# tiberiu44/TTS-Cube

Hardware: AMD Instinct MI355X
Metric: audio samples/sec (HiFi-GAN vocoder inference) (higher is better)
Workload: dtype f32 (split fp16 hi/lo x3 MFMA, fp32 accumulate)

## Files before the change

include/ttscube_hip.h:

```cpp
#ifndef TTSCUBE_HIP_H
#define TTSCUBE_HIP_H

#include <stddef.h>
#include <stdint.h>

#ifdef __cplusplus
extern "C" {
#endif

#define TTSC_OK 0
#define TTSC_EINVAL (-1)
#define TTSC_EHIP (-2)
#define TTSC_ESTATE (-3)
#define TTSC_ENOMEM (-4)
#define TTSC_ERANGE (-5)

const char* ttsc_version(void);
const char* ttsc_last_error(void);
int ttsc_device_count(void);

typedef struct ttsc_conv1d ttsc_conv1d;

typedef struct {
    int32_t in_channels;
// ... 18 lines not shown
    const float* gate_dev;
    float gate_slope;
} ttsc_conv1d_epilogue;

int ttsc_conv1d_create(const ttsc_conv1d_cfg* cfg, ttsc_conv1d** out);
int ttsc_conv1d_set_weight(ttsc_conv1d* c, const float* weight_host, const float* bias_host);
int ttsc_conv1d_set_weight_device(ttsc_conv1d* c, const float* weight_dev, const float* bias_dev, void* stream);
int ttsc_conv1d_set_weight_device_dgrad(ttsc_conv1d* c, const float* fwd_weight_dev, void* stream);
int ttsc_conv1d_set_precision(ttsc_conv1d* c, int32_t precision);
int64_t ttsc_conv1d_out_len(const ttsc_conv1d* c, int64_t Lin);
int32_t ttsc_conv1d_in_channels(const ttsc_conv1d* c);
int ttsc_conv1d_set_activation_scale(ttsc_conv1d* c, float scale);
float ttsc_conv1d_get_activation_scale(const ttsc_conv1d* c);
int ttsc_conv1d_set_nonfinite_flag(ttsc_conv1d* c, uint32_t* flag_dev);
int ttsc_absmax(const float* x_dev, int64_t n, float* out_dev, void* stream);
int ttsc_conv1d_forward(const ttsc_conv1d* c, const float* x_dev, int32_t B, int64_t Lin, float* y_dev,
                        const float* resid_dev, const ttsc_conv1d_epilogue* ep, void* stream);
int ttsc_conv1d_forward_ragged(const ttsc_conv1d* c, const float* x_dev, int32_t B, int64_t Lin, float* y_dev,
                               const float* resid_dev, const ttsc_conv1d_epilogue* ep, const int32_t* in_len_dev,
                               const int32_t* out_len_dev, void* stream);
int ttsc_conv1d_forward_pitched(const ttsc_conv1d* c, const float* x_dev, int32_t B, int64_t Lin, float* y_dev,
                                const float* resid_dev, const ttsc_conv1d_epilogue* ep, const int32_t* in_len_dev,
                                const int32_t* out_len_dev, int64_t Lout_pitch, void* stream);
int ttsc_respair_supported(const ttsc_conv1d* conv1, const ttsc_conv1d* conv2);
int ttsc_respair_forward(const ttsc_conv1d* conv1, const ttsc_conv1d* conv2, const float* x_dev, int32_t B, int64_t L,
                         float* y_dev, int32_t accumulate, const int32_t* len_dev, void* stream);
int ttsc_rbchain_supported(const ttsc_conv1d* const* convs1, const ttsc_conv1d* const* convs2, int32_t npairs);
int ttsc_rbchain_forward(const ttsc_conv1d* const* convs1, const ttsc_conv1d* const* convs2, int32_t npairs, const float* x_dev,
                         int32_t B, int64_t L, float* y_dev, int32_t accumulate, const int32_t* len_dev, int32_t tile_shape,
                         void* stream);
int ttsc_rbchain_post_supported(const ttsc_conv1d* const* convs1, const ttsc_conv1d* const* convs2, int32_t npairs, const ttsc_conv1d* post);
int ttsc_rbchain_post_forward(const ttsc_conv1d* const* convs1, const ttsc_conv1d* const* convs2, int32_t npairs, const float* x_dev, int32_t B,
                              int64_t L, const float* ysum_dev, const ttsc_conv1d* post, const ttsc_conv1d_epilogue* post_ep, float* wav_dev,
                              const int32_t* len_dev, void* stream);
void ttsc_conv1d_destroy(ttsc_conv1d* c);

int ttsc_weight_norm_forward(const float* v_dev, const float* g_dev, float* w_dev, float* norm_dev, int32_t rows, int64_t cols, void* stream);
int ttsc_weight_norm_backward(const float* dw_dev, const float* v_dev, const float* g_dev, const float* norm_dev, float* dv_dev,
                              float* dg_dev, int32_t rows, int64_t cols, void* stream);
size_t ttsc_matvec_workspace_bytes(int32_t rows, int64_t cols);
int ttsc_matvec(const float* w_dev, int32_t rows, int64_t cols, const float* x_dev, int32_t transpose, float* out_dev, void* ws_dev, size_t ws_bytes,
                void* stream);
int ttsc_l2_normalize(const float* x_dev, int32_t n, float eps, float* out_dev, float* norm_dev, void* stream);
size_t ttsc_dot_workspace_bytes(int64_t n);
int ttsc_dot(const float* a_dev, const float* b_dev, int64_t n, float* out_dev, void* ws_dev, size_t ws_bytes, void* stream);
int ttsc_div_scalar(const float* w_dev, const float* sigma_dev, float* out_dev, int64_t n, void* stream);
// ... 334 lines not shown
```

ttscube_amd/_lib.py:

```python
import ctypes as C
import os

_HERE = os.path.dirname(os.path.abspath(__file__))
LIB_PATH = os.path.join(_HERE, 'csrc', 'libttscube_hip.so')


class TTSCError(RuntimeError):
    pass


class Conv1dCfg(C.Structure):
    _fields_ = [('in_channels', C.c_int32), ('out_channels', C.c_int32), ('kernel_size', C.c_int32),
                ('stride', C.c_int32), ('padding', C.c_int32), ('dilation', C.c_int32), ('transposed', C.c_int32), ('groups', C.c_int32)]


class Conv1dEpilogue(C.Structure):
    _fields_ = [('in_scale', C.c_float), ('in_slope', C.c_float), ('out_scale', C.c_float),
                ('out_act', C.c_int32), ('accumulate', C.c_int32), ('gate_dev', C.c_void_p), ('gate_slope', C.c_float)]


MAX_UPS, MAX_RB, MAX_DIL = 8, 8, 8


class WBankEntry(C.Structure):
# ... 44 lines not shown
    'ttsc_device_count': (C.c_int, []),
    'ttsc_conv1d_create': (C.c_int, [C.POINTER(Conv1dCfg), C.POINTER(C.c_void_p)]),
    'ttsc_conv1d_set_weight': (C.c_int, [C.c_void_p, C.c_void_p, C.c_void_p]),
    'ttsc_conv1d_set_precision': (C.c_int, [C.c_void_p, C.c_int32]),
    'ttsc_conv1d_out_len': (C.c_int64, [C.c_void_p, C.c_int64]),
    'ttsc_conv1d_set_activation_scale': (C.c_int, [C.c_void_p, C.c_float]),
    'ttsc_conv1d_get_activation_scale': (C.c_float, [C.c_void_p]),
    'ttsc_absmax': (C.c_int, [C.c_void_p, C.c_int64, C.c_void_p, C.c_void_p]),
    'ttsc_hifigan_calibrate': (C.c_int, [C.c_void_p, C.c_void_p, C.c_int32, C.c_int64, C.c_void_p, C.c_void_p, C.c_size_t, C.c_void_p]),
    'ttsc_hifigan_get_activation_scale': (C.c_int, [C.c_void_p, C.c_char_p, C.POINTER(C.c_float)]),
    'ttsc_hifigan_set_activation_scales': (C.c_int, [C.c_void_p, C.POINTER(C.c_char_p), C.POINTER(C.c_float), C.c_int32]),
    'ttsc_hifigan_recalibrations': (C.c_int32, [C.c_void_p]),
    'ttsc_hifigan_set_branch_streams': (C.c_int, [C.c_void_p, C.c_void_p, C.c_void_p]),
    'ttsc_hifigan_set_range_check': (C.c_int, [C.c_void_p, C.c_int32]),
    'ttsc_hifigan_range_status': (C.c_int32, [C.c_void_p, C.c_void_p]),
    'ttsc_conv1d_set_nonfinite_flag': (C.c_int, [C.c_void_p, C.c_void_p]),
    'ttsc_conv1d_in_channels': (C.c_int32, [C.c_void_p]),
    'ttsc_conv1d_forward': (C.c_int, [C.c_void_p, C.c_void_p, C.c_int32, C.c_int64, C.c_void_p, C.c_void_p,
                                      C.POINTER(Conv1dEpilogue), C.c_void_p]),
    'ttsc_conv1d_forward_ragged': (C.c_int, [C.c_void_p, C.c_void_p, C.c_int32, C.c_int64, C.c_void_p, C.c_void_p,
                                             C.POINTER(Conv1dEpilogue), C.c_void_p, C.c_void_p, C.c_void_p]),
    'ttsc_conv1d_forward_pitched': (C.c_int, [C.c_void_p, C.c_void_p, C.c_int32, C.c_int64, C.c_void_p, C.c_void_p,
                                              C.POINTER(Conv1dEpilogue), C.c_void_p, C.c_void_p, C.c_int64, C.c_void_p]),
    'ttsc_rbchain_supported': (C.c_int, [C.POINTER(C.c_void_p), C.POINTER(C.c_void_p), C.c_int32]),
    'ttsc_rbchain_forward': (C.c_int, [C.POINTER(C.c_void_p), C.POINTER(C.c_void_p), C.c_int32, C.c_void_p, C.c_int32, C.c_int64,
                                       C.c_void_p, C.c_int32, C.c_void_p, C.c_int32, C.c_void_p]),
    'ttsc_rbchain_post_supported': (C.c_int, [C.POINTER(C.c_void_p), C.POINTER(C.c_void_p), C.c_int32, C.c_void_p]),
    'ttsc_rbchain_post_forward': (C.c_int, [C.POINTER(C.c_void_p), C.POINTER(C.c_void_p), C.c_int32, C.c_void_p, C.c_int32, C.c_int64, C.c_void_p,
                                            C.c_void_p, C.POINTER(Conv1dEpilogue), C.c_void_p, C.c_void_p, C.c_void_p]),
    'ttsc_respair_supported': (C.c_int, [C.c_void_p, C.c_void_p]),
    'ttsc_respair_forward': (C.c_int, [C.c_void_p, C.c_void_p, C.c_void_p, C.c_int32, C.c_int64, C.c_void_p, C.c_int32,
                                       C.c_void_p, C.c_void_p]),
    'ttsc_conv1d_destroy': (None, [C.c_void_p]),
    'ttsc_conv1d_set_weight_device': (C.c_int, [C.c_void_p, C.c_void_p, C.c_void_p, C.c_void_p]),
    'ttsc_conv_wgrad_grouped': (C.c_int, [C.c_void_p, C.c_void_p, C.c_void_p, C.c_int32, C.c_int32, C.c_int32, C.c_int32, C.c_int64, C.c_int64,
                                          C.c_int32, C.c_int32, C.c_int32, C.c_float, C.c_float, C.c_void_p, C.c_size_t, C.c_void_p]),
    'ttsc_conv_wgrad': (C.c_int, [C.c_void_p, C.c_void_p, C.c_void_p, C.c_int32, C.c_int32, C.c_int32, C.c_int64, C.c_int64,
                                  C.c_int32, C.c_int32, C.c_int32, C.c_float, C.c_float, C.c_void_p, C.c_size_t, C.c_void_p]),
    'ttsc_conv1d_set_weight_device_dgrad': (C.c_int, [C.c_void_p, C.c_void_p, C.c_void_p]),
    'ttsc_weight_norm_forward': (C.c_int, [C.c_void_p, C.c_void_p, C.c_void_p, C.c_void_p, C.c_int32, C.c_int64, C.c_void_p]),
    'ttsc_weight_norm_backward': (C.c_int, [C.c_void_p, C.c_void_p, C.c_void_p, C.c_void_p, C.c_void_p, C.c_void_p, C.c_int32,
                                            C.c_int64, C.c_void_p]),
    'ttsc_matvec_workspace_bytes': (C.c_size_t, [C.c_int32, C.c_int64]),
    'ttsc_matvec': (C.c_int, [C.c_void_p, C.c_int32, C.c_int64, C.c_void_p, C.c_int32, C.c_void_p, C.c_void_p, C.c_size_t, C.c_void_p]),
    'ttsc_rows_segment_sum': (C.c_int, [C.c_void_p, C.c_void_p, C.c_void_p, C.c_int64, C.c_int32, C.c_int32, C.c_void_p]),
    'ttsc_l2_normalize': (C.c_int, [C.c_void_p, C.c_int32, C.c_float, C.c_void_p, C.c_void_p, C.c_void_p]),
# ... 356 lines not shown
```

ttscube_amd/csrc/conv1d.hip:

```cpp
#include <climits>
#include <cmath>
#include <cstdlib>
#include <type_traits>

#include "common.hpp"
#include "conv_kernels.hpp"

namespace ttsc {

static constexpr unsigned LEAN_OOB = 0x80000000u;
__device__ __forceinline__ float lean_load(__amdgpu_buffer_rsrc_t rs, unsigned voff, int soff) {
    return __uint_as_float(__builtin_amdgcn_raw_buffer_load_b32(rs, (int)voff, soff, 0));
}

template <int C, int K, int D, bool LEAN>
__global__ __launch_bounds__(256, 2) void conv_f16x3_wide_kernel(ConvArgs a) {
    extern __shared__ __attribute__((aligned(16))) char smem_raw[];
    constexpr int WM = 2, WN = 2;
    constexpr int MI = 2, NJ = 4, NT = WN * NJ * 32;
    constexpr int SPAN = NT + (K - 1) * D;
    constexpr int SPANP = (SPAN + 63) & ~63;
    constexpr int BUFSZ = 4 * SPAN + 2;
    constexpr int NCHUNK = C / 16, COTN = C / 32;
    constexpr int AITEMS = WM * MI * 2 * 64;
    half8* Xp = reinterpret_cast<half8*>(smem_raw);
    half8* Aw = Xp + 2 * BUFSZ;
    const int tid = threadIdx.x, lane = tid & 63, wave = tid >> 6;
    const int wm = wave / WN, wn = wave % WN;
    const int half = lane >> 5, l31 = lane & 31;
    const int b = blockIdx.z;
    const int q0 = blockIdx.x * NT;
    const int lin = a.in_len ? a.in_len[b] : a.Lin;
    if (a.out_len && q0 >= a.out_len[b]) return;
    const int cotg = blockIdx.y * (WM * MI);
#ifdef TTSC_ABLATE
    const unsigned wg_lin = blockIdx.x + gridDim.x * (blockIdx.y + gridDim.y * blockIdx.z);
#endif
    TTSC_STAMP(a, wg_lin, 0);
    TTSC_STAMP_HWID(a, wg_lin, 15);

    f32x16 acc[MI][NJ];
    const float* ai_first = a.acc_init ? (a.resid ? a.resid : (a.accumulate ? a.y : nullptr)) : nullptr;
    const float* ai_second = (a.acc_init && a.resid && a.accumulate) ? a.y : nullptr;
    const unsigned ai_L = (unsigned)a.Lout;
    const unsigned ai_row0 = ((unsigned)b * a.Cout + (cotg + wm * MI) * 32 + 4 * half) * ai_L;
// ... 41 lines not shown
#pragma unroll
                        for (int r = 0; r < 16; ++r) acc[i][n0 + n][r] += t[n][r];
                }
        }
        if (a.bias) {
#pragma unroll
            for (int i = 0; i < MI; ++i) {
                float bv[16];
#pragma unroll
                for (int r = 0; r < 16; ++r) bv[r] = a.bias[(cotg + wm * MI + i) * 32 + (r & 3) + 8 * (r >> 2) + 4 * half];
#pragma unroll
                for (int n = 0; n < NJ; ++n)
#pragma unroll
                    for (int r = 0; r < 16; ++r) acc[i][n][r] += bv[r];
            }
        }
#pragma unroll
        for (int i = 0; i < MI; ++i)
#pragma unroll
            for (int n = 0; n < NJ; ++n)
#pragma unroll
                for (int r = 0; r < 16; ++r) acc[i][n][r] *= inv;
    };
    if (a.acc_init) {
    } else if (a.epi_prefetch && a.bias && (a.resid || a.accumulate)) {
        const float inv = 1.f / a.w_unscale;
#pragma unroll
        for (int i = 0; i < MI; ++i)
#pragma unroll
            for (int r = 0; r < 16; ++r) {
                const float bv = a.bias[(cotg + wm * MI + i) * 32 + (r & 3) + 8 * (r >> 2) + 4 * half] * inv;
#pragma unroll
                for (int j = 0; j < NJ; ++j) acc[i][j][r] = bv;
            }
    } else {
#pragma unroll
        for (int i = 0; i < MI; ++i)
#pragma unroll
            for (int j = 0; j < NJ; ++j)
#pragma unroll
                for (int r = 0; r < 16; ++r) acc[i][j][r] = 0.f;
    }

    const float* xb = a.x + (size_t)b * C * a.Lin;
    const int lo = q0 - D * ((K - 1) / 2);
    const half8* wsrc = reinterpret_cast<const half8*>(a.wph) + (size_t)cotg * 128 + lane;
    if (a.skew) {
// ... 9 lines not shown
        for (int i = 0; i < AITEMS / 64 / 4; ++i) {
            const int blk = wave + i * 4;
            __builtin_amdgcn_global_load_lds((const __attribute__((address_space(1))) void*)(wj + blk * 64),
                                             (__attribute__((address_space(3))) void*)(Aw + slot * AITEMS + blk * 64), 16, 0, 0);
        }
    };

    constexpr int XIT = (2 * SPANP + 255) / 256;
    static_assert(XIT <= K, "one staging item per tap");
    float xr[XIT][8];
    unsigned xoff[XIT];
    int xslot[XIT];
    bool xok[XIT];
#pragma unroll
    for (int e = 0; e < XIT; ++e) {
        const int i = tid + e * 256;
        const int h = i >= SPANP ? 1 : 0;
        const int p = i - h * SPANP;
        const int pos = lo + p;
        xok[e] = pos >= 0 && pos < lin;
        int pc = pos > lin - 1 ? lin - 1 : pos;
        pc = pc < 0 ? 0 : pc;
        xoff[e] = (unsigned)(h * 8 * a.Lin + pc);
        xslot[e] = (p < SPAN && i < 2 * SPANP) ? (h * 2) * SPAN + p : 4 * SPAN;
        if (LEAN) xoff[e] = (xok[e] && xslot[e] < 4 * SPAN) ? xoff[e] * 4u : LEAN_OOB;
    }
    const __amdgpu_buffer_rsrc_t xrs = __builtin_amdgcn_make_buffer_rsrc(const_cast<float*>(xb), 0, LEAN ? C * a.Lin * 4 : 0, 0x00020000);
    const int xrow = a.Lin * 4;
    auto x_issue_item = [&](int e, int c) __attribute__((always_inline)) {
        if constexpr (LEAN) {
            const int s0 = c * 16 * xrow;
#pragma unroll
            for (int ch = 0; ch < 8; ++ch) xr[e][ch] = lean_load(xrs, xoff[e], s0 + ch * xrow);
        } else {
            const float* rc = xb + (size_t)(c * 16) * a.Lin;
#pragma unroll
            for (int ch = 0; ch < 8; ++ch) xr[e][ch] = rc[(size_t)ch * a.Lin + xoff[e]];
        }
    };
    auto x_commit_item = [&](int e, half8* buf) __attribute__((always_inline)) {
        typedef unsigned u32x4 __attribute__((ext_vector_type(4)));
        u32x4 uh, ul;
#pragma unroll
        for (int ch = 0; ch < 8; ch += 2) {
            float v0 = (LEAN || xok[e]) ? xr[e][ch] * a.in_scale : 0.f, v1 = (LEAN || xok[e]) ? xr[e][ch + 1] * a.in_scale : 0.f;
            v0 = fmaxf(v0, v0 * a.in_slope);
            v1 = fmaxf(v1, v1 * a.in_slope);
            unsigned h, l;
            split2_f16(v0, v1, h, l);
            uh[ch >> 1] = h;
            ul[ch >> 1] = l;
        }
        const half8 vh = __builtin_bit_cast(half8, uh), vl = __builtin_bit_cast(half8, ul);
        buf[xslot[e]] = vh;
        buf[xslot[e] + (xslot[e] < 4 * SPAN ? SPAN : 1)] = vl;
    };

    const half8* xbase = Xp + (unsigned)((half * 2) * SPAN + wn * (NJ * 32) + l31);
    const half8* abase = Aw + (unsigned)(wm * (MI * 128) + lane);
    auto chunk = [&](int c, auto buf_tag, auto par_tag) __attribute__((always_inline)) {
        constexpr int BUF = decltype(buf_tag)::value;
        constexpr int PAR = decltype(par_tag)::value;
        half8* nxt = Xp + (1 - BUF) * BUFSZ;
#pragma unroll
        for (int j = 0; j < K; ++j) {
            const int slot = (PAR + j) & 1;
            if (j + 1 < K)
                stage_A(c, j + 1, slot ^ 1);
            else
                stage_A(c + 1 < NCHUNK ? c + 1 : c, 0, slot ^ 1);
            __builtin_amdgcn_sched_barrier(0);
            half8 ah[MI], al[MI], bh[NJ], bl[NJ];
#pragma unroll
            for (int i = 0; i < MI; ++i) {
                ah[i] = abase[slot * AITEMS + i * 128];
                al[i] = abase[slot * AITEMS + i * 128 + 64];
            }
#pragma unroll
            for (int n = 0; n < NJ; ++n) {
                bh[n] = xbase[BUF * BUFSZ + j * D + n * 32];
                bl[n] = xbase[BUF * BUFSZ + SPAN + j * D + n * 32];
            }
            const int e = K - 1 - j;
            if (e < XIT && !TTSC_DBG(a, 1)) {
                x_commit_item(e, nxt);
                x_issue_item(e, c + 2 < NCHUNK ? c + 2 : NCHUNK - 1);
            }
#pragma unroll
            for (int i = 0; i < MI; ++i)
#pragma unroll
                for (int n = 0; n < NJ; ++n) acc[i][n] = __builtin_amdgcn_mfma_f32_32x32x16_f16(al[i], bh[n], acc[i][n], 0, 0, 0);
#pragma unroll
            for (int i = 0; i < MI; ++i)
#pragma unroll
                for (int n = 0; n < NJ; ++n) acc[i][n] = __builtin_amdgcn_mfma_f32_32x32x16_f16(ah[i], bl[n], acc[i][n], 0, 0, 0);
#pragma unroll
            for (int i = 0; i < MI; ++i)
#pragma unroll
                for (int n = 0; n < NJ; ++n) acc[i][n] = __builtin_amdgcn_mfma_f32_32x32x16_f16(ah[i], bh[n], acc[i][n], 0, 0, 0);
            __builtin_amdgcn_sched_barrier(0);
            if (!TTSC_DBG(a, 2)) __syncthreads();
        }
    };

    stage_A(0, 0, 0);
#pragma unroll
    for (int e = 0; e < XIT; ++e) x_issue_item(e, 0);
    if (a.acc_init) {
        __builtin_amdgcn_sched_barrier(0);
        acc_load_first(0);
        __builtin_amdgcn_sched_barrier(0);
    }
#pragma unroll
    for (int e = 0; e < XIT; ++e) x_commit_item(e, Xp);
#pragma unroll
    for (int e = 0; e < XIT; ++e) x_issue_item(e, 1);
    if (a.acc_init) {
        __builtin_amdgcn_sched_barrier(0);
#pragma unroll
        for (int i = 1; i < MI; ++i) acc_load_first(i);
        acc_init_finish();
    }
    __syncthreads();
    TTSC_STAMP(a, wg_lin, 1);
    for (int c = 0; c < NCHUNK; c += 2) {
        chunk(c, std::integral_constant<int, 0>(), std::integral_constant<int, 0>());
        chunk(c + 1, std::integral_constant<int, 1>(), std::integral_constant<int, (K & 1)>());
    }
    TTSC_STAMP(a, wg_lin, 2);

    if (TTSC_DBG(a, 4)) {
        float t = 0.f;
#pragma unroll
        for (int i = 0; i < MI; ++i)
#pragma unroll
            for (int n = 0; n < NJ; ++n) t += acc[i][n][0] + acc[i][n][7];
        if (t == 12345.678f) a.y[0] = 1.f;
        return;
    }
    if (a.acc_init) {
#pragma unroll
        for (int i = 0; i < MI; ++i)
#pragma unroll
            for (int n = 0; n < NJ; ++n) {
                const int q = q0 + wn * (NJ * 32) + n * 32 + l31;
                if (q < a.Lout) {
                    float* yp = a.y + ((size_t)b * a.Cout + (cotg + wm * MI + i) * 32 + 4 * half) * a.Lout + q;
#pragma unroll
                    for (int r = 0; r < 16; ++r) yp[(size_t)((r & 3) + 8 * (r >> 2)) * a.Lout] = acc[i][n][r] * a.w_unscale;
                }
            }
    } else if (a.epi_prefetch && (a.resid || a.accumulate)) {
        const float* rsrc = a.resid;
        const float* ysrc = a.accumulate ? a.y : nullptr;
        constexpr int NTILE = MI * NJ;
        const unsigned L1 = (unsigned)a.Lout;
        const unsigned row0 = ((unsigned)b * a.Cout + (cotg + wm * MI) * 32 + 4 * half) * L1;
        const int qw = q0 + wn * (NJ * 32) + l31;
        auto tile_off = [&](int t) __attribute__((always_inline)) -> unsigned {
            const int i = t / NJ, n = t % NJ;
            const int q = qw + n * 32;
            return row0 + (unsigned)(i * 32) * L1 + (unsigned)(q < a.Lout ? q : 0);
        };
// ... 333 lines not shown
    } else {
#pragma unroll
        for (int e = 0; e < 4; ++e)
            if (q + e < a.Lout) yb[q + e] = res[e];
    }
}

template <int MI, int NJ, int TMAX>
static int launch_f16_t(const ConvArgs& a, int B, hipStream_t s) {
    constexpr int NT = 4 * NJ * 32;
    constexpr int MT = MI * 32;
    dim3 grid((unsigned)ceil_div(a.q_cnt, NT), (unsigned)(a.CoutP / MT), (unsigned)B);
    const size_t lds = (size_t)a.span_pad * 4 * 16 + (size_t)a.ntaps * MI * 2 * 64 * 16;
    if (int rc = ensure_full_lds((const void*)conv_f16x3_kernel<MI, NJ, TMAX>)) return rc;
    hipLaunchKernelGGL((conv_f16x3_kernel<MI, NJ, TMAX>), grid, dim3(256), lds, s, a);
    hipError_t e = hipGetLastError();
    if (e != hipSuccess) {
        set_error("conv_f16x3_kernel launch failed: %s", hipGetErrorString(e));
        return TTSC_EHIP;
    }
    return TTSC_OK;
}

template <int C, int K, int D, bool LEAN>
static int launch_f16_wide_l(const ConvArgs& a0, int B, hipStream_t s) {
    constexpr int NT = 256;
    constexpr int SPAN = NT + (K - 1) * D;
    dim3 grid((unsigned)ceil_div(a0.Lout, NT), (unsigned)(C / 128), (unsigned)B);
    ConvArgs a = a0;
    static const int skew_env = getenv("TTSC_CONV_SKEW") ? atoi(getenv("TTSC_CONV_SKEW")) : 0;
    a.skew = ((size_t)grid.x * grid.y * grid.z >= 1024) ? skew_env : 0;
    static const int epi_env = getenv("TTSC_CONV_EPI_PREFETCH") ? atoi(getenv("TTSC_CONV_EPI_PREFETCH")) : 1;
    a.epi_prefetch = (epi_env && !a.gate && a.out_act == TTSC_ACT_NONE && a.Cout == C && (size_t)B * C * a.Lout < (1ull << 32)) ? 1 : 0;
    constexpr size_t lds = (size_t)2 * (4 * SPAN + 2) * 16 + (size_t)2 * (2 * 2 * 2 * 64) * 16;
    if (int rc = ensure_full_lds((const void*)conv_f16x3_wide_kernel<C, K, D, LEAN>)) return rc;
    hipLaunchKernelGGL((conv_f16x3_wide_kernel<C, K, D, LEAN>), grid, dim3(256), lds, s, a);
    hipError_t e = hipGetLastError();
    if (e != hipSuccess) {
        set_error("conv_f16x3_wide_kernel launch failed: %s", hipGetErrorString(e));
        return TTSC_EHIP;
    }
    return TTSC_OK;
}

template <int C, int K, int D>
static int launch_f16_wide(const ConvArgs& a, int B, hipStream_t s) {
    return a.lean ? launch_f16_wide_l<C, K, D, true>(a, B, s) : launch_f16_wide_l<C, K, D, false>(a, B, s);
}


template <int CIN, int J, int MI, int NJ, bool LEAN>
__global__ __launch_bounds__(256, 2) void conv_f16x3_tall_kernel(ConvArgs a) {
    extern __shared__ __attribute__((aligned(16))) char smem_raw[];
    constexpr int WM = 2, WN = 2, NT = WN * NJ * 32;
    constexpr int SPAN = NT + (J - 1);
    constexpr int SPANP = (SPAN + 63) & ~63;
    constexpr int BUFSZ = 4 * SPAN + 2;
    constexpr int NCHUNK = CIN / 16;
    constexpr int AITEMS = WM * MI * 2 * 64;
    static_assert(NCHUNK % 2 == 0, "slot parity: chunks in pairs (two chunks of NTAPS taps each end on the slot they started on)");
    half8* Xp = reinterpret_cast<half8*>(smem_raw);
    half8* Aw = Xp + 2 * BUFSZ;
    const int tid = threadIdx.x, lane = tid & 63, wave = tid >> 6;
    const int wm = wave / WN, wn = wave % WN;
    const int half = lane >> 5, l31 = lane & 31;
    int bx, by, bz;
    if (a.swz_nx > 0) {
        const unsigned id = blockIdx.x, xcd = id & 7u, u = id >> 3;
        by = (int)(u % (unsigned)a.swz_ny);
// ... 676 lines not shown
    __syncthreads();
    if (threadIdx.x == 0) atomicMax(out, __float_as_uint(fmaxf(fmaxf(red[0], red[1]), fmaxf(red[2], red[3]))));
}
}

extern "C" int ttsc_absmax(const float* x_dev, int64_t n, float* out_dev, void* stream) {
    TTSC_REQUIRE(x_dev && out_dev && n > 0, "ttsc_absmax: bad argument");
    const int blocks = (int)std::min<int64_t>((n / 4 + 255) / 256 + 1, 1024);
    hipLaunchKernelGGL(absmax_kernel, dim3(blocks), dim3(256), 0, (hipStream_t)stream, x_dev, (long)n, reinterpret_cast<unsigned*>(out_dev));
    hipError_t e = hipGetLastError();
    if (e != hipSuccess) {
        set_error("absmax_kernel launch failed: %s", hipGetErrorString(e));
        return TTSC_EHIP;
    }
    return TTSC_OK;
}

extern "C" int ttsc_conv1d_forward_ragged(const ttsc_conv1d* c, const float* x, int32_t B, int64_t Lin, float* y,
                                          const float* resid, const ttsc_conv1d_epilogue* ep, const int32_t* in_len_dev,
                                          const int32_t* out_len_dev, void* stream) {
    return ttsc_conv1d_forward_pitched(c, x, B, Lin, y, resid, ep, in_len_dev, out_len_dev, 0, stream);
}

extern "C" int ttsc_conv1d_forward_pitched(const ttsc_conv1d* c, const float* x, int32_t B, int64_t Lin, float* y,
                                           const float* resid, const ttsc_conv1d_epilogue* ep, const int32_t* in_len_dev,
                                           const int32_t* out_len_dev, int64_t Lout_pitch, void* stream) {
    TTSC_REQUIRE(c && x && y, "ttsc_conv1d_forward: null argument");
    TTSC_REQUIRE(Lout_pitch == 0 || (Lout_pitch > 0 && in_len_dev && out_len_dev),
                 "ttsc_conv1d_forward_pitched: an output pitch needs per-utterance lengths (in_len_dev, out_len_dev)");
    if (!c->has_weight) {
        set_error("ttsc_conv1d_forward: weights not set");
        return TTSC_ESTATE;
    }
    TTSC_REQUIRE(B > 0 && Lin > 0, "ttsc_conv1d_forward: bad B/Lin (%d, %lld)", B, (long long)Lin);
    TTSC_REQUIRE(!ep || (ep->in_slope >= 0.f && ep->in_slope <= 1.f), "ttsc_conv1d_forward: in_slope must be in [0,1]");
    const auto& g = c->cfg;
    const int64_t Lout = Lout_pitch > 0 ? Lout_pitch : ttsc_conv1d_out_len(c, Lin);
    TTSC_REQUIRE(Lout > 0, "ttsc_conv1d_forward: output length %lld <= 0", (long long)Lout);
    TTSC_REQUIRE(Lin < (1ll << 30) && Lout < (1ll << 30), "ttsc_conv1d_forward: length too large");
    hipStream_t s = (hipStream_t)stream;
    for (const auto& ph : c->phases) {
        ConvArgs a;
        a.x = x;
        a.y = y;
        a.resid = resid;
        a.nf_flag = nullptr;
        a.wp = ph.wp_dev;
        a.wph = ph.wph_dev;
        a.w_unscale = c->w_unscale;
        a.bias = (c->dev_weights && c->bias_ext) ? c->bias_ext : c->bias_dev;
        a.in_len = in_len_dev;
        a.out_len = out_len_dev;
        a.dbg = 0;
        a.skew = 0;
        a.acc_init = 0;
        a.epi_prefetch = 0;
        a.swz_nx = a.swz_ny = 0;
        a.lean = 0;
        a.short_from = INT_MAX;
        a.fold_S = a.fold_B = 0;
        a.amax_x = a.amax_w = nullptr;
        a.amax_out = nullptr;
#ifdef TTSC_ABLATE
        if (const char* ev = getenv("TTSC_CONV_DBG")) a.dbg = atoi(ev);
        a.prof = nullptr;
        if (const char* ev = getenv("TTSC_PROF_PTR")) a.prof = reinterpret_cast<unsigned long long*>(strtoull(ev, nullptr, 0));
#endif
        a.vphase = c->vfused ? ((c->vrow4 && c->precision == TTSC_PREC_F16X3) ? -4 : g.out_channels) : 0;
        if (a.vphase == -4) {
            TTSC_REQUIRE(!(ep && ep->gate_dev), "ttsc_conv1d_forward: the gate epilogue is not available on this transposed layer");
            TTSC_REQUIRE(((uintptr_t)y % 16 == 0) && (!resid || (uintptr_t)resid % 16 == 0), "ttsc_conv1d_forward: y / resid must be 16-byte aligned for ConvTranspose1d(k=4, s=4)");
        }
        a.Cin = c->groups > 1 ? c->cin_tile : g.in_channels;
        a.CinTot = g.in_channels;
        a.groups = c->groups;
        a.cin_g = c->cin_g;
        a.cout_g = c->cout_g;
        a.CinP = c->CinP;
        a.Cout = g.out_channels;
        a.CoutP = c->CoutP;
        a.Lin = (int)Lin;
// ... 18 lines not shown
            if (qhi <= qlo) continue;
            a.q_lo = (int)qlo;
            a.q_cnt = (int)(qhi - qlo);
        }
        const int last = (ph.ntaps - 1) * ph.tap_step;
        a.min_shift = ph.tap_base + (last < 0 ? last : 0);
        a.span = c->NT + (last < 0 ? -last : last);
        a.span_pad = a.span + 1;
        a.in_scale = ep ? ep->in_scale : 1.f;
        const float* w_plain = c->dev_weights ? c->w_plain_ext : c->w_plain_dev;
        const bool use_cout1 = !g.transposed && c->groups == 1 && g.out_channels == 1 && g.in_channels <= 64 && g.kernel_size <= 16 && g.dilation == 1 &&
                               w_plain && !(ep && ep->gate_dev);
        if (c->precision == TTSC_PREC_F16X3 && !use_cout1) {
            a.in_scale *= c->act_scale;
            a.w_unscale = c->w_unscale / c->act_scale;
        }
        a.in_slope = ep ? ep->in_slope : 1.f;
        a.out_scale = ep ? ep->out_scale : 1.f;
        a.out_act = ep ? ep->out_act : TTSC_ACT_NONE;
        a.accumulate = ep ? ep->accumulate : 0;
        a.gate = ep ? ep->gate_dev : nullptr;
        a.gate_slope = ep ? ep->gate_slope : 1.f;
        int rc;
        if (use_cout1) {
            a.wp = w_plain;
            a.nf_flag = c->nf_flag;
            dim3 grid((unsigned)ceil_div(Lout, 1024), (unsigned)B);
            hipLaunchKernelGGL(conv_cout1_kernel, grid, dim3(256), 0, s, a);
            hipError_t e = hipGetLastError();
            if (e != hipSuccess) {
                set_error("conv_cout1_kernel launch failed: %s", hipGetErrorString(e));
                return TTSC_EHIP;
            }
            rc = TTSC_OK;
        } else if (c->precision == TTSC_PREC_F16X3) {
            const int nt = c->MT >= 64 ? 256 : 512;
            a.span = nt + (last < 0 ? -last : last);
            a.span_pad = a.span;
            TTSC_REQUIRE(ph.ntaps <= 16, "f16x3 path supports at most 16 taps per phase (got %d)", ph.ntaps);
            auto wgs16 = [&](int mt, int nt) { return (long)ceil_div(a.q_cnt, nt) * (c->CoutP / mt) * B; };
            auto set_nt16 = [&](int n) {
                a.span = n + (last < 0 ? -last : last);
                a.span_pad = a.span;
            };
            static const bool big_only = getenv("TTSC_F16_TILE") && atoi(getenv("TTSC_F16_TILE")) == 0;
            const char* wide_ev = getenv("TTSC_CONV_WIDE");
            const int wide_env = wide_ev ? atoi(wide_ev) : 1;
            const long want16 = 512;
            const bool wide_shape = !g.transposed && !a.gate && g.in_channels == g.out_channels &&
                                    (g.out_channels == 128 || g.out_channels == 256) &&
                                    ((g.kernel_size == 3 || g.kernel_size == 7 || g.kernel_size == 11)
#ifdef TTSC_PROBE_EVENK
                                     || ((g.kernel_size == 4 || g.kernel_size == 6) && g.dilation == 1)
#endif
                                     ) &&
                                    (g.dilation == 1 || g.dilation == 3 || g.dilation == 5) &&
                                    g.padding == g.dilation * (g.kernel_size - 1) / 2;
            static const int acc_init_env = getenv("TTSC_CONV_ACC_INIT") ? atoi(getenv("TTSC_CONV_ACC_INIT")) : 1;
            a.acc_init = (acc_init_env && wide_env && wide_shape && a.out_act == TTSC_ACT_NONE && a.out_scale == 1.f && c->CoutP == g.out_channels &&
                          (size_t)B * g.out_channels * Lout < (1ull << 32)) ? 1 : 0;
            static const bool tall_on = !(getenv("TTSC_CONV_TALL") && atoi(getenv("TTSC_CONV_TALL")) == 0);
            const bool tall0 = g.in_channels == 512 && ph.ntaps == 4 && c->CoutP % 256 == 0;
            const bool tall1 = g.in_channels == 256 && ph.ntaps == 6 && c->CoutP % 128 == 0;
            const bool tall_shape = tall_on && c->vfused && a.vphase > 0 && !a.gate && c->CinP == g.in_channels && (tall0 || tall1);
            const char* lean_ev = getenv("TTSC_CONV_LEAN");
            a.lean = (!(lean_ev && atoi(lean_ev) == 0) && (int64_t)g.in_channels * Lin * 4 < (1ll << 31) && a.in_scale > 0.f && std::isfinite(a.in_scale)) ? 1 : 0;
            if (tall_shape && (tall0 ? 256 : 128) == g.out_channels) a.short_from = g.kernel_size - (ph.ntaps - 1) * g.stride;
            if (tall_shape && (wide_env == 2 || (long)ceil_div(a.q_cnt, tall0 ? 128 : 256) * (c->CoutP / (tall0 ? 256 : 128)) * B >= want16)) {
                rc = tall0 ? launch_f16_tall<512, 4, 4, 2>(a, B, s) : launch_f16_tall<256, 6, 2, 4>(a, B, s);
            } else if (wide_env && wide_shape && (wide_env == 2 || (long)ceil_div(a.Lout, 256) * (g.out_channels / 128) * B >= want16)) {
                if (g.out_channels == 256)
                    rc = launch_f16_wide_k<256>(a, B, g.dilation, s);
                else
                    rc = launch_f16_wide_k<128>(a, B, g.dilation, s);
            } else if (c->MT >= 64) {
                if (big_only || wgs16(64, 256) >= want16)
                    rc = launch_f16<2, 2>(a, B, s);
                else if (wgs16(64, 128) >= want16) {
                    set_nt16(128);
                    rc = launch_f16<2, 1>(a, B, s);
                } else {
                    set_nt16(128);
                    rc = launch_f16<1, 1>(a, B, s);
                }
            } else {
                if (big_only || wgs16(32, 512) >= want16)
                    rc = launch_f16<1, 4>(a, B, s);
                else if (wgs16(32, 256) >= want16) {
                    set_nt16(256);
                    rc = launch_f16<1, 2>(a, B, s);
                } else {
                    set_nt16(128);
                    rc = launch_f16<1, 1>(a, B, s);
// ... 90 lines not shown
```

ttscube_amd/csrc/conv_kernels.hpp:

```cpp
#pragma once
#include "common.hpp"
#include "conv_internal.hpp"

namespace ttsc {

typedef float f32x16 __attribute__((ext_vector_type(16)));

#ifdef TTSC_ABLATE
#define TTSC_DBG(args, bit) (((args).dbg & (bit)) != 0)
#define TTSC_STAMP(args, wg, i)                                                                              \
    do {                                                                                                     \
        if ((args).prof && threadIdx.x == 0) (args).prof[(size_t)(wg) * 24 + (i)] = __builtin_amdgcn_s_memrealtime(); \
    } while (0)
#define TTSC_STAMP_HWID(args, wg, i)                                                                         \
    do {                                                                                                     \
        if ((args).prof && threadIdx.x == 0) {                                                               \
            unsigned hw, xcc;                                                                                \
            asm volatile("s_getreg_b32 %0, hwreg(HW_REG_HW_ID)" : "=s"(hw));                                 \
            asm volatile("s_getreg_b32 %0, hwreg(HW_REG_XCC_ID)" : "=s"(xcc));                               \
            (args).prof[(size_t)(wg) * 24 + (i)] = ((unsigned long long)(xcc & 0xf) << 32) | hw;            \
        }                                                                                                    \
    } while (0)
#else
#define TTSC_DBG(args, bit) false
// ... 8 lines not shown
    float* y;
    const float* resid;
    const float* wp;
    const void* wph;
    float w_unscale;
    const float* bias;
    const int* in_len;
    const int* out_len;
    int Cin, CinP, Cout, CoutP;
    int CinTot;
    int groups, cin_g, cout_g;
    int Lin, Lout;
    int ntaps, tap_base, tap_step;
    int out_stride, out_off;
    int q_lo, q_cnt;
    int span, span_pad, min_shift;
    float in_scale, in_slope, out_scale;
    int out_act, accumulate;
    int vphase;
    int acc_init;
    int epi_prefetch;
    int swz_nx, swz_ny;
    int lean;
    int short_from;
    int skew;
    int dbg;
#ifdef TTSC_ABLATE
    unsigned long long* prof;
#endif
    unsigned* nf_flag;
    const float* gate;
    float gate_slope;
    int fold_S, fold_B;
    const float* amax_x;
    const float* amax_w;
    unsigned* amax_out;
};

__device__ __forceinline__ float pow2_to(float m, int target) {
    const int ex = (int)((__float_as_uint(m) >> 23) & 0xffu);
    if (ex == 0 || ex == 255) return 1.f;
    int s = target - (ex - 126);
    s = s > 100 ? 100 : (s < -100 ? -100 : s);
    return __uint_as_float((unsigned)(127 + s) << 23);
}
int launch_amax2(const float* x, long nx, float* out_x, const float* w, long nw, float* out_w, hipStream_t s, bool prezeroed = false);
// ... 532 lines not shown
```

Before: 292.4 million.

## Add interleaved-column layout to wide f16x3 conv for 128-bit accumulate epilogue

Adds an IL variant of the wide conv kernel. Each lane owns four adjacent output columns, and the LDS input tile is stored in a column-interleaved plane layout, so the accumulate-init load and the final store become 128-bit buffer ops instead of scalar ones. The variant is enabled by default when the conv takes the wide lean path with acc_init, K is 3, 7 or 11, and alignment holds; TTSC_CONV_WIDE_IL=0 turns it off. A query entry point reports whether the path is taken. The cost is a larger LDS footprint, more registers for the staged tiles, and s_nop padding between stores.

```diff
diff --git a/include/ttscube_hip.h b/include/ttscube_hip.h
--- a/include/ttscube_hip.h
+++ b/include/ttscube_hip.h
@@ -64,6 +64,8 @@
 int ttsc_conv1d_forward_pitched(const ttsc_conv1d* c, const float* x_dev, int32_t B, int64_t Lin, float* y_dev,
                                 const float* resid_dev, const ttsc_conv1d_epilogue* ep, const int32_t* in_len_dev,
                                 const int32_t* out_len_dev, int64_t Lout_pitch, void* stream);
+int ttsc_conv1d_wide_il_taken(const ttsc_conv1d* c, const float* x_dev, int32_t B, int64_t Lin, float* y_dev, const float* resid_dev,
+                              const ttsc_conv1d_epilogue* ep, const int32_t* in_len_dev, const int32_t* out_len_dev, int64_t Lout_pitch);
 int ttsc_respair_supported(const ttsc_conv1d* conv1, const ttsc_conv1d* conv2);
 int ttsc_respair_forward(const ttsc_conv1d* conv1, const ttsc_conv1d* conv2, const float* x_dev, int32_t B, int64_t L,
                          float* y_dev, int32_t accumulate, const int32_t* len_dev, void* stream);
diff --git a/ttscube_amd/_lib.py b/ttscube_amd/_lib.py
--- a/ttscube_amd/_lib.py
+++ b/ttscube_amd/_lib.py
@@ -90,6 +90,8 @@
                                              C.POINTER(Conv1dEpilogue), C.c_void_p, C.c_void_p, C.c_void_p]),
     'ttsc_conv1d_forward_pitched': (C.c_int, [C.c_void_p, C.c_void_p, C.c_int32, C.c_int64, C.c_void_p, C.c_void_p,
                                               C.POINTER(Conv1dEpilogue), C.c_void_p, C.c_void_p, C.c_int64, C.c_void_p]),
+    'ttsc_conv1d_wide_il_taken': (C.c_int, [C.c_void_p, C.c_void_p, C.c_int32, C.c_int64, C.c_void_p, C.c_void_p,
+                                            C.POINTER(Conv1dEpilogue), C.c_void_p, C.c_void_p, C.c_int64]),
     'ttsc_rbchain_supported': (C.c_int, [C.POINTER(C.c_void_p), C.POINTER(C.c_void_p), C.c_int32]),
     'ttsc_rbchain_forward': (C.c_int, [C.POINTER(C.c_void_p), C.POINTER(C.c_void_p), C.c_int32, C.c_void_p, C.c_int32, C.c_int64,
                                        C.c_void_p, C.c_int32, C.c_void_p, C.c_int32, C.c_void_p]),
diff --git a/ttscube_amd/csrc/conv1d.hip b/ttscube_amd/csrc/conv1d.hip
--- a/ttscube_amd/csrc/conv1d.hip
+++ b/ttscube_amd/csrc/conv1d.hip
@@ -5,22 +5,29 @@
 
 #include "common.hpp"
 #include "conv_kernels.hpp"
+#include "conv_wide_layout.hpp"
 
 namespace ttsc {
 
 static constexpr unsigned LEAN_OOB = 0x80000000u;
+typedef float f32x4 __attribute__((ext_vector_type(4)));
+typedef unsigned u32x4 __attribute__((ext_vector_type(4)));
 __device__ __forceinline__ float lean_load(__amdgpu_buffer_rsrc_t rs, unsigned voff, int soff) {
     return __uint_as_float(__builtin_amdgcn_raw_buffer_load_b32(rs, (int)voff, soff, 0));
 }
 
-template <int C, int K, int D, bool LEAN>
+template <int C, int K, int D, bool LEAN, bool IL = false>
 __global__ __launch_bounds__(256, 2) void conv_f16x3_wide_kernel(ConvArgs a) {
+    static_assert(!IL || LEAN, "interleaved columns come with the lean staging pass only");
     extern __shared__ __attribute__((aligned(16))) char smem_raw[];
     constexpr int WM = 2, WN = 2;
     constexpr int MI = 2, NJ = 4, NT = WN * NJ * 32;
     constexpr int SPAN = NT + (K - 1) * D;
     constexpr int SPANP = (SPAN + 63) & ~63;
-    constexpr int BUFSZ = 4 * SPAN + 2;
+    static_assert(NT == wide_il::NT && SPAN == wide_il::span(K, D), "conv_wide_layout.hpp describes this tile");
+    constexpr int PLANE = IL ? wide_il::plane(K, D) : SPAN;
+    constexpr int DUMP = 4 * PLANE;
+    constexpr int BUFSZ = DUMP + 2;
     constexpr int NCHUNK = C / 16, COTN = C / 32;
     constexpr int AITEMS = WM * MI * 2 * 64;
     half8* Xp = reinterpret_cast<half8*>(smem_raw);
@@ -108,7 +115,57 @@
 #pragma unroll
                 for (int r = 0; r < 16; ++r) acc[i][n][r] *= inv;
     };
-    if (a.acc_init) {
+    const int wm_s = __builtin_amdgcn_readfirstlane(wave) / WN;
+    const int il_rowb = a.Lout * 4;
+    const int il_s0 = (cotg + wm_s * MI) * 32 * il_rowb;
+    const int il_col = q0 + wn * (NJ * 32) + NJ * l31;
+    const unsigned il_voff = il_col < a.Lout ? (unsigned)(4 * half * a.Lout + il_col) * 4u : LEAN_OOB;
+    const __amdgpu_buffer_rsrc_t il_yrs = __builtin_amdgcn_make_buffer_rsrc(a.y + (size_t)b * C * a.Lout, 0, IL ? C * a.Lout * 4 : 0, 0x00020000);
+    const __amdgpu_buffer_rsrc_t il_frs =
+        __builtin_amdgcn_make_buffer_rsrc(const_cast<float*>(ai_first ? ai_first : a.y) + (size_t)b * C * a.Lout, 0, IL ? C * a.Lout * 4 : 0, 0x00020000);
+    auto il_soff = [&](int i, int r) __attribute__((always_inline)) -> int { return il_s0 + (i * 32 + (r & 3) + 8 * (r >> 2)) * il_rowb; };
+    f32x4 il_t[MI][16];
+    auto il_load_first = [&](int i) __attribute__((always_inline)) {
+        if (ai_first) {
+#pragma unroll
+            for (int r = 0; r < 16; ++r) il_t[i][r] = __builtin_bit_cast(f32x4, __builtin_amdgcn_raw_buffer_load_b128(il_frs, (int)il_voff, il_soff(i, r), 0));
+        } else {
+#pragma unroll
+            for (int r = 0; r < 16; ++r) il_t[i][r] = f32x4{0.f, 0.f, 0.f, 0.f};
+        }
+    };
+    auto il_finish = [&]() __attribute__((always_inline)) {
+        const float inv = 1.f / a.w_unscale;
+        if (ai_second) {
+#pragma unroll
+            for (int i = 0; i < MI; ++i)
+#pragma unroll
+                for (int r0 = 0; r0 < 16; r0 += 8) {
+                    f32x4 t[8];
+#pragma unroll
+                    for (int r = 0; r < 8; ++r) t[r] = __builtin_bit_cast(f32x4, __builtin_amdgcn_raw_buffer_load_b128(il_yrs, (int)il_voff, il_soff(i, r0 + r), 0));
+#pragma unroll
+                    for (int r = 0; r < 8; ++r) il_t[i][r0 + r] += t[r];
+                }
+        }
+        if (a.bias) {
+#pragma unroll
+            for (int i = 0; i < MI; ++i) {
+                float bv[16];
+#pragma unroll
+                for (int r = 0; r < 16; ++r) bv[r] = a.bias[(cotg + wm * MI + i) * 32 + (r & 3) + 8 * (r >> 2) + 4 * half];
+#pragma unroll
+                for (int r = 0; r < 16; ++r) il_t[i][r] += bv[r];
+            }
+        }
+#pragma unroll
+        for (int i = 0; i < MI; ++i)
+#pragma unroll
+            for (int n = 0; n < NJ; ++n)
+#pragma unroll
+                for (int r = 0; r < 16; ++r) acc[i][n][r] = il_t[i][r][n] * inv;
+    };
+    if (IL || a.acc_init) {
     } else if (a.epi_prefetch && a.bias && (a.resid || a.accumulate)) {
         const float inv = 1.f / a.w_unscale;
 #pragma unroll
@@ -164,8 +221,8 @@
         int pc = pos > lin - 1 ? lin - 1 : pos;
         pc = pc < 0 ? 0 : pc;
         xoff[e] = (unsigned)(h * 8 * a.Lin + pc);
-        xslot[e] = (p < SPAN && i < 2 * SPANP) ? (h * 2) * SPAN + p : 4 * SPAN;
-        if (LEAN) xoff[e] = (xok[e] && xslot[e] < 4 * SPAN) ? xoff[e] * 4u : LEAN_OOB;
+        xslot[e] = (p < SPAN && i < 2 * SPANP) ? (h * 2) * PLANE + (IL ? wide_il::slot(K, D, p) : p) : DUMP;
+        if (LEAN) xoff[e] = (xok[e] && xslot[e] < DUMP) ? xoff[e] * 4u : LEAN_OOB;
     }
     const __amdgpu_buffer_rsrc_t xrs = __builtin_amdgcn_make_buffer_rsrc(const_cast<float*>(xb), 0, LEAN ? C * a.Lin * 4 : 0, 0x00020000);
     const int xrow = a.Lin * 4;
@@ -195,10 +252,10 @@
         }
         const half8 vh = __builtin_bit_cast(half8, uh), vl = __builtin_bit_cast(half8, ul);
         buf[xslot[e]] = vh;
-        buf[xslot[e] + (xslot[e] < 4 * SPAN ? SPAN : 1)] = vl;
+        buf[xslot[e] + (xslot[e] < DUMP ? PLANE : 1)] = vl;
     };
 
-    const half8* xbase = Xp + (unsigned)((half * 2) * SPAN + wn * (NJ * 32) + l31);
+    const half8* xbase = Xp + (unsigned)((half * 2) * PLANE + wn * (IL ? 32 : NJ * 32) + l31);
     const half8* abase = Aw + (unsigned)(wm * (MI * 128) + lane);
     auto chunk = [&](int c, auto buf_tag, auto par_tag) __attribute__((always_inline)) {
         constexpr int BUF = decltype(buf_tag)::value;
@@ -220,8 +277,9 @@
             }
 #pragma unroll
             for (int n = 0; n < NJ; ++n) {
-                bh[n] = xbase[BUF * BUFSZ + j * D + n * 32];
-                bl[n] = xbase[BUF * BUFSZ + SPAN + j * D + n * 32];
+                const int fo = IL ? wide_il::frag(K, D, n, j) : j * D + n * 32;
+                bh[n] = xbase[BUF * BUFSZ + fo];
+                bl[n] = xbase[BUF * BUFSZ + PLANE + fo];
             }
             const int e = K - 1 - j;
             if (e < XIT && !TTSC_DBG(a, 1)) {
@@ -248,7 +306,11 @@
     stage_A(0, 0, 0);
 #pragma unroll
     for (int e = 0; e < XIT; ++e) x_issue_item(e, 0);
-    if (a.acc_init) {
+    if constexpr (IL) {
+        __builtin_amdgcn_sched_barrier(0);
+        il_load_first(0);
+        __builtin_amdgcn_sched_barrier(0);
+    } else if (a.acc_init) {
         __builtin_amdgcn_sched_barrier(0);
         acc_load_first(0);
         __builtin_amdgcn_sched_barrier(0);
@@ -257,7 +319,12 @@
     for (int e = 0; e < XIT; ++e) x_commit_item(e, Xp);
 #pragma unroll
     for (int e = 0; e < XIT; ++e) x_issue_item(e, 1);
-    if (a.acc_init) {
+    if constexpr (IL) {
+        __builtin_amdgcn_sched_barrier(0);
+#pragma unroll
+        for (int i = 1; i < MI; ++i) il_load_first(i);
+        il_finish();
+    } else if (a.acc_init) {
         __builtin_amdgcn_sched_barrier(0);
 #pragma unroll
         for (int i = 1; i < MI; ++i) acc_load_first(i);
@@ -280,7 +347,17 @@
         if (t == 12345.678f) a.y[0] = 1.f;
         return;
     }
-    if (a.acc_init) {
+    if constexpr (IL) {
+#pragma unroll
+        for (int i = 0; i < MI; ++i)
+#pragma unroll
+            for (int r = 0; r < 16; ++r) {
+                const f32x4 v = {acc[i][0][r] * a.w_unscale, acc[i][1][r] * a.w_unscale, acc[i][2][r] * a.w_unscale, acc[i][3][r] * a.w_unscale};
+                __builtin_amdgcn_raw_buffer_store_b128(__builtin_bit_cast(u32x4, v), il_yrs, (int)il_voff, il_soff(i, r), 0);
+                asm volatile("s_nop 3" ::: "memory");
+                __builtin_amdgcn_sched_barrier(0);
+            }
+    } else if (a.acc_init) {
 #pragma unroll
         for (int i = 0; i < MI; ++i)
 #pragma unroll
@@ -660,7 +737,7 @@
     return TTSC_OK;
 }
 
-template <int C, int K, int D, bool LEAN>
+template <int C, int K, int D, bool LEAN, bool IL = false>
 static int launch_f16_wide_l(const ConvArgs& a0, int B, hipStream_t s) {
     constexpr int NT = 256;
     constexpr int SPAN = NT + (K - 1) * D;
@@ -670,9 +747,10 @@
     a.skew = ((size_t)grid.x * grid.y * grid.z >= 1024) ? skew_env : 0;
     static const int epi_env = getenv("TTSC_CONV_EPI_PREFETCH") ? atoi(getenv("TTSC_CONV_EPI_PREFETCH")) : 1;
     a.epi_prefetch = (epi_env && !a.gate && a.out_act == TTSC_ACT_NONE && a.Cout == C && (size_t)B * C * a.Lout < (1ull << 32)) ? 1 : 0;
-    constexpr size_t lds = (size_t)2 * (4 * SPAN + 2) * 16 + (size_t)2 * (2 * 2 * 2 * 64) * 16;
-    if (int rc = ensure_full_lds((const void*)conv_f16x3_wide_kernel<C, K, D, LEAN>)) return rc;
-    hipLaunchKernelGGL((conv_f16x3_wide_kernel<C, K, D, LEAN>), grid, dim3(256), lds, s, a);
+    constexpr size_t lds = (size_t)2 * (IL ? wide_il::bufsz(K, D) : 4 * SPAN + 2) * 16 + (size_t)2 * (2 * 2 * 2 * 64) * 16;
+    static_assert(2 * lds <= 160 * 1024, "two workgroups per CU");
+    if (int rc = ensure_full_lds((const void*)conv_f16x3_wide_kernel<C, K, D, LEAN, IL>)) return rc;
+    hipLaunchKernelGGL((conv_f16x3_wide_kernel<C, K, D, LEAN, IL>), grid, dim3(256), lds, s, a);
     hipError_t e = hipGetLastError();
     if (e != hipSuccess) {
         set_error("conv_f16x3_wide_kernel launch failed: %s", hipGetErrorString(e));
@@ -683,6 +761,7 @@
 
 template <int C, int K, int D>
 static int launch_f16_wide(const ConvArgs& a, int B, hipStream_t s) {
+    if (a.il) return launch_f16_wide_l<C, K, D, true, true>(a, B, s);
     return a.lean ? launch_f16_wide_l<C, K, D, true>(a, B, s) : launch_f16_wide_l<C, K, D, false>(a, B, s);
 }
 
@@ -1405,9 +1484,34 @@
     return ttsc_conv1d_forward_pitched(c, x, B, Lin, y, resid, ep, in_len_dev, out_len_dev, 0, stream);
 }
 
+static bool wide_il_rule(const ConvArgs& a, bool wide_launch, int C, int K) {
+    const char* ev = getenv("TTSC_CONV_WIDE_IL");
+    return wide_launch && a.lean && a.acc_init && (K == 3 || K == 7 || K == 11) && a.Lout % 4 == 0 && (uintptr_t)a.y % 16 == 0 &&
+           (!a.resid || (uintptr_t)a.resid % 16 == 0) && (int64_t)C * a.Lout * 4 < (1ll << 31) && !(ev && atoi(ev) == 0);
+}
+
+static int conv1d_forward_impl(const ttsc_conv1d* c, const float* x, int32_t B, int64_t Lin, float* y, const float* resid,
+                               const ttsc_conv1d_epilogue* ep, const int32_t* in_len_dev, const int32_t* out_len_dev, int64_t Lout_pitch,
+                               void* stream, int* il_query);
+
 extern "C" int ttsc_conv1d_forward_pitched(const ttsc_conv1d* c, const float* x, int32_t B, int64_t Lin, float* y,
                                            const float* resid, const ttsc_conv1d_epilogue* ep, const int32_t* in_len_dev,
                                            const int32_t* out_len_dev, int64_t Lout_pitch, void* stream) {
+    return conv1d_forward_impl(c, x, B, Lin, y, resid, ep, in_len_dev, out_len_dev, Lout_pitch, stream, nullptr);
+}
+
+extern "C" int ttsc_conv1d_wide_il_taken(const ttsc_conv1d* c, const float* x, int32_t B, int64_t Lin, float* y, const float* resid,
+                                         const ttsc_conv1d_epilogue* ep, const int32_t* in_len_dev, const int32_t* out_len_dev,
+                                         int64_t Lout_pitch) {
+    int taken = 0;
+    if (conv1d_forward_impl(c, x, B, Lin, y, resid, ep, in_len_dev, out_len_dev, Lout_pitch, nullptr, &taken) != TTSC_OK) return 0;
+    return taken;
+}
+
+static int conv1d_forward_impl(const ttsc_conv1d* c, const float* x, int32_t B, int64_t Lin, float* y, const float* resid,
+                               const ttsc_conv1d_epilogue* ep, const int32_t* in_len_dev, const int32_t* out_len_dev, int64_t Lout_pitch,
+                               void* stream, int* il_query) {
+    if (il_query) *il_query = 0;
     TTSC_REQUIRE(c && x && y, "ttsc_conv1d_forward: null argument");
     TTSC_REQUIRE(Lout_pitch == 0 || (Lout_pitch > 0 && in_len_dev && out_len_dev),
                  "ttsc_conv1d_forward_pitched: an output pitch needs per-utterance lengths (in_len_dev, out_len_dev)");
@@ -1440,6 +1544,7 @@
         a.epi_prefetch = 0;
         a.swz_nx = a.swz_ny = 0;
         a.lean = 0;
+        a.il = 0;
         a.short_from = INT_MAX;
         a.fold_S = a.fold_B = 0;
         a.amax_x = a.amax_w = nullptr;
@@ -1504,6 +1609,7 @@
         a.gate = ep ? ep->gate_dev : nullptr;
         a.gate_slope = ep ? ep->gate_slope : 1.f;
         int rc;
+        if (il_query && (use_cout1 || c->precision != TTSC_PREC_F16X3)) return TTSC_OK;
         if (use_cout1) {
             a.wp = w_plain;
             a.nf_flag = c->nf_flag;
@@ -1548,9 +1654,16 @@
             const char* lean_ev = getenv("TTSC_CONV_LEAN");
             a.lean = (!(lean_ev && atoi(lean_ev) == 0) && (int64_t)g.in_channels * Lin * 4 < (1ll << 31) && a.in_scale > 0.f && std::isfinite(a.in_scale)) ? 1 : 0;
             if (tall_shape && (tall0 ? 256 : 128) == g.out_channels) a.short_from = g.kernel_size - (ph.ntaps - 1) * g.stride;
-            if (tall_shape && (wide_env == 2 || (long)ceil_div(a.q_cnt, tall0 ? 128 : 256) * (c->CoutP / (tall0 ? 256 : 128)) * B >= want16)) {
+            const bool tall_launch = tall_shape && (wide_env == 2 || (long)ceil_div(a.q_cnt, tall0 ? 128 : 256) * (c->CoutP / (tall0 ? 256 : 128)) * B >= want16);
+            const bool wide_launch = !tall_launch && wide_env && wide_shape && (wide_env == 2 || (long)ceil_div(a.Lout, 256) * (g.out_channels / 128) * B >= want16);
+            a.il = wide_il_rule(a, wide_launch, g.out_channels, g.kernel_size) ? 1 : 0;
+            if (il_query) {
+                *il_query = a.il;
+                return TTSC_OK;
+            }
+            if (tall_launch) {
                 rc = tall0 ? launch_f16_tall<512, 4, 4, 2>(a, B, s) : launch_f16_tall<256, 6, 2, 4>(a, B, s);
-            } else if (wide_env && wide_shape && (wide_env == 2 || (long)ceil_div(a.Lout, 256) * (g.out_channels / 128) * B >= want16)) {
+            } else if (wide_launch) {
                 if (g.out_channels == 256)
                     rc = launch_f16_wide_k<256>(a, B, g.dilation, s);
                 else
diff --git a/ttscube_amd/csrc/conv_kernels.hpp b/ttscube_amd/csrc/conv_kernels.hpp
--- a/ttscube_amd/csrc/conv_kernels.hpp
+++ b/ttscube_amd/csrc/conv_kernels.hpp
@@ -54,6 +54,7 @@
     int epi_prefetch;
     int swz_nx, swz_ny;
     int lean;
+    int il;
     int short_from;
     int skew;
     int dbg;
diff --git a/ttscube_amd/csrc/conv_wide_layout.hpp b/ttscube_amd/csrc/conv_wide_layout.hpp
--- /dev/null
+++ b/ttscube_amd/csrc/conv_wide_layout.hpp
@@ -0,0 +1,46 @@
+#pragma once
+
+namespace ttsc {
+namespace wide_il {
+
+constexpr int NT = 256;
+constexpr int span(int K, int D) { return NT + (K - 1) * D; }
+constexpr int pitch(int K, int D) {
+    const int q = (span(K, D) + 3) / 4;
+    return q + ((2 - q % 4) + 4) % 4;
+}
+constexpr int plane(int K, int D) { return 4 * pitch(K, D); }
+constexpr int dump(int K, int D) { return 4 * plane(K, D); }
+constexpr int bufsz(int K, int D) { return dump(K, D) + 2; }
+constexpr int slot(int K, int D, int p) { return (p & 3) * pitch(K, D) + (p >> 2); }
+constexpr int frag(int K, int D, int n, int j) { return ((n + j * D) & 3) * pitch(K, D) + ((n + j * D) >> 2); }
+
+constexpr bool check(int K, int D) {
+    const int S = span(K, D), PQ = pitch(K, D), PL = plane(K, D);
+    if (PQ % 4 != 2 || 4 * PQ < S) return false;
+    for (int p = 0; p < S; ++p) {
+        const int s = slot(K, D, p);
+        if (s < 0 || s >= PL) return false;
+        if ((s % PQ) * 4 + s / PQ != p) return false;
+    }
+    for (int p0 = 0; p0 + 8 <= S; p0 += 8) {
+        unsigned seen = 0;
+        for (int e = 0; e < 8; ++e) seen |= 1u << (slot(K, D, p0 + e) % 8);
+        if (seen != 0xffu) return false;
+    }
+    for (int wn = 0; wn < 2; ++wn)
+        for (int l31 = 0; l31 < 32; ++l31)
+            for (int n = 0; n < 4; ++n)
+                for (int j = 0; j < K; ++j) {
+                    const int p = 4 * l31 + n + j * D + wn * 128;
+                    if (p >= S) return false;
+                    if (wn * 32 + l31 + frag(K, D, n, j) != slot(K, D, p)) return false;
+                }
+    return true;
+}
+static_assert(check(3, 1) && check(3, 3) && check(3, 5), "wide IL layout, K = 3");
+static_assert(check(7, 1) && check(7, 3) && check(7, 5), "wide IL layout, K = 7");
+static_assert(check(11, 1) && check(11, 3) && check(11, 5), "wide IL layout, K = 11");
+
+}
+}
```

Result: no change. 294.3 million, median of 6 (+0.7%).
